# arpg/Kangaroo

Measured on AMD Instinct MI355X. Metric: kinectfusion_frames_per_sec_640x480_to_512cubed_tsdf, higher is better.
Workload: dtype f32

## Files before the change

include/kfx_debug.h:

```cpp
#ifndef KFX_DEBUG_H
#define KFX_DEBUG_H

#include "kfx.h"

#ifdef __cplusplus
extern "C" {
#endif

int kfx_debug_rmw(const kfx_volume* vol, int variant, kfx_stream stream);

int kfx_debug_div_uniform_check(float b, unsigned long long* d_out, kfx_stream stream);

int kfx_debug_div_core_check(unsigned seed, int per_divisor, unsigned long long* d_out, kfx_stream stream);
int kfx_debug_sqrt_core_check(unsigned long long* d_out, kfx_stream stream);
int kfx_debug_wave_xor_check(unsigned seed, unsigned long long* d_out, kfx_stream stream);

int kfx_debug_summary_export(kfx_sdf_summary* s, float tol, float vref, int fine_shift, void* R_out, void* C_out, int dims_out[12],
                             kfx_stream stream);


#ifdef __cplusplus
}
#endif
#endif
```

kangaroo_amd/csrc/debug.hip:

```cpp
#include "kfx_device.h"
#include "sampling.h"
#include "../../include/kfx_debug.h"

namespace kfx {

__global__ __launch_bounds__(256) void k_rmw_linear(float4* __restrict__ base, size_t n4)
{
    const size_t stride = (size_t)gridDim.x * blockDim.x;
    for (size_t i = (size_t)blockIdx.x * blockDim.x + threadIdx.x; i < n4; i += stride) {
        float4 c = base[i];
        c.y += 1.0f;
        c.w += 1.0f;
        base[i] = c;
    }
}

template <int ZC>
__global__ __launch_bounds__(256) void k_rmw_brick(unsigned char* vptr, size_t pitch, size_t img_pitch, int X, int Y, int Z)
{
    const int tid = threadIdx.x, lane = tid & 63, wv = tid >> 6;
    const int x0 = (blockIdx.x * 32 + (lane & 31)) * 2;
    const int y = blockIdx.y * 8 + wv * 2 + (lane >> 5);
    const int zbeg = blockIdx.z * ZC, zend = min(zbeg + ZC, Z);
    if (x0 >= X || y >= Y) return;
// ... 173 lines not shown
    hipLaunchKernelGGL(k_div_core_check, dim3(4096), dim3(256), 0, (hipStream_t)stream, seed, per_divisor, d_out);
    return check_launch("kfx_debug_div_core_check");
}

extern "C" int kfx_debug_sqrt_core_check(unsigned long long* d_out, kfx_stream stream)
{
    if (!d_out) return set_error(KFX_E_NULL, "kfx_debug_sqrt_core_check");
    hipLaunchKernelGGL(k_sqrt_core_check, dim3(4096), dim3(256), 0, (hipStream_t)stream, d_out);
    return check_launch("kfx_debug_sqrt_core_check");
}

extern "C" int kfx_debug_div_uniform_check(float b, unsigned long long* d_out, kfx_stream stream)
{
    if (!d_out) return set_error(KFX_E_NULL, "kfx_debug_div_uniform_check");
    if (!div_uniform_safe_host(b)) return set_error(KFX_E_RANGE, "kfx_debug_div_uniform_check: divisor outside [2^-40, 2^40]");
    hipLaunchKernelGGL(k_div_uniform_check, dim3(256), dim3(256), 0, (hipStream_t)stream, b, 1.0f / b, d_out);
    return check_launch("kfx_debug_div_uniform_check");
}

extern "C" int kfx_debug_rmw(const kfx_volume* vol, int variant, kfx_stream stream)
{
    if (!vol || !vol->ptr) return set_error(KFX_E_NULL, "kfx_debug_rmw");
    hipStream_t s = (hipStream_t)stream;
    const int X = (int)vol->w, Y = (int)vol->h, Z = (int)vol->d;
    unsigned char* p = (unsigned char*)vol->ptr;
    switch (variant) {
    case 0: {
        const size_t n4 = ((vol->d - 1) * vol->img_pitch + (vol->h - 1) * vol->pitch + vol->w * 8) / 16;
        hipLaunchKernelGGL(k_rmw_linear, dim3(256 * 8), dim3(256), 0, s, (float4*)p, n4);
        break;
    }
    case 1: hipLaunchKernelGGL(k_rmw_brick<16>, dim3(ceil_div(X, 64), ceil_div(Y, 8), ceil_div(Z, 16)), dim3(256), 0, s, p, vol->pitch, vol->img_pitch, X, Y, Z); break;
    case 2: hipLaunchKernelGGL(k_rmw_rows<16>, dim3(ceil_div(X, 128), ceil_div(Y, 4), ceil_div(Z, 16)), dim3(256), 0, s, p, vol->pitch, vol->img_pitch, X, Y, Z); break;
    case 3: hipLaunchKernelGGL(k_rmw_column, dim3(ceil_div(X, 128), ceil_div(Y, 4), 1), dim3(256), 0, s, p, vol->pitch, vol->img_pitch, X, Y, Z); break;
    case 4: hipLaunchKernelGGL(k_rmw_brick<64>, dim3(ceil_div(X, 64), ceil_div(Y, 8), ceil_div(Z, 64)), dim3(256), 0, s, p, vol->pitch, vol->img_pitch, X, Y, Z); break;
    case 5: hipLaunchKernelGGL(k_rmw_rows<4>, dim3(ceil_div(X, 128), ceil_div(Y, 4), ceil_div(Z, 4)), dim3(256), 0, s, p, vol->pitch, vol->img_pitch, X, Y, Z); break;
#define GEN(ID, WX, WY, ZC, NT) \
    case ID: hipLaunchKernelGGL((k_rmw_gen<WX, WY, ZC, NT>), dim3(ceil_div(X, 128 * WX), ceil_div(Y, WY), ceil_div(Z, ZC)), dim3(256), 0, s, p, vol->pitch, vol->img_pitch, X, Y, Z); break;
    GEN(10, 4, 1, 16, false)
    GEN(11, 2, 2, 16, false)
    GEN(12, 1, 4, 16, false)
    GEN(13, 1, 4, 16, true)
    GEN(14, 4, 1, 16, true)
    GEN(15, 1, 4, 1, false)
    GEN(16, 1, 4, 64, false)
    GEN(17, 4, 1, 4, false)
    GEN(18, 2, 2, 16, true)
#undef GEN
    default: return set_error(KFX_E_RANGE, "kfx_debug_rmw: variant");
    }
    return check_launch("kfx_debug_rmw");
}

extern "C" int kfx_debug_summary_export(kfx_sdf_summary* s, float tol, float vref, int fine_shift, void* R_out, void* C_out, int dims_out[12],
                                        kfx_stream stream)
{
    if (!s || !dims_out) return set_error(KFX_E_NULL, "kfx_debug_summary_export: null argument");
    if (fine_shift < 3 || fine_shift > 5) return set_error(KFX_E_RANGE, "kfx_debug_summary_export: fine_shift in [3, 5]");
    ClassView cv;
    summary_class_layout(s, fine_shift, cv);
    dims_out[0] = s->nbx; dims_out[1] = s->nby; dims_out[2] = s->nbz;
    dims_out[3] = cv.fine.first; dims_out[4] = cv.fine.rw; dims_out[5] = cv.fine.ny;
    dims_out[6] = cv.coarse.first; dims_out[7] = cv.coarse.rw; dims_out[8] = cv.coarse.ny;
    dims_out[9] = cv.words; dims_out[10] = s->n_coarse; dims_out[11] = (s->h_skippable && s->builds) ? ((volatile int*)s->h_skippable)[(s->builds - 1) % KFX_SUMMARY_RING] : -2;
    const size_t n = (size_t)s->nbx * s->nby * s->nbz;
    hipStream_t st = (hipStream_t)stream;
    if (R_out && hipMemcpyAsync(R_out, s->R, n * sizeof(float4), hipMemcpyDeviceToDevice, st) != hipSuccess) return set_error(KFX_E_RANGE, "kfx_debug_summary_export: copy");
    if (C_out) {
        if (int e = summary_classes_prepare(s, tol, vref, fine_shift, st)) return e;
        if (hipMemcpyAsync(C_out, s->C, (size_t)cv.words * sizeof(unsigned), hipMemcpyDeviceToDevice, st) != hipSuccess || hipStreamSynchronize(st) != hipSuccess)
            return set_error(KFX_E_RANGE, "kfx_debug_summary_export: copy");
        dims_out[11] = (s->h_skippable && s->builds) ? ((volatile int*)s->h_skippable)[(s->builds - 1) % KFX_SUMMARY_RING] : -2;
    }
    return 0;
}
```

kangaroo_amd/csrc/host_args.h:

```cpp
#pragma once

#include <cstdio>
#include <cstdlib>

#include "kfx_device.h"

namespace kfx {

constexpr size_t VOLUME_MAX_DIM = 65535, VOLUME_ANY_DIM = ~(size_t)0;

inline int check_volume(const kfx_volume* vol, size_t cell_bytes, size_t min_dim, size_t max_dim, const char* what)
{
    auto fail = [what](int code, const char* rule) {
        char msg[160];
        snprintf(msg, sizeof(msg), "%s: %s", what, rule);
        return set_error(code, msg);
    };
    if (!vol || !vol->ptr) return fail(KFX_E_NULL, "null volume");
    if (vol->w < min_dim || vol->h < min_dim || vol->d < min_dim || vol->w > max_dim || vol->h > max_dim || vol->d > max_dim)
        return fail(KFX_E_SHAPE, "volume dimensions");
    if (vol->pitch < vol->w * cell_bytes || vol->img_pitch < vol->pitch * (vol->h - 1) + vol->w * cell_bytes)
        return fail(KFX_E_SHAPE, "volume pitch smaller than a row / slice");
    if (((uintptr_t)vol->ptr | vol->pitch | vol->img_pitch) & (cell_bytes - 1)) return fail(KFX_E_ALIGN, "volume not aligned to its cell size");
    return 0;
}

inline kfx_volume slab_full_volume(const kfx_volume* vol, const kfx_slab* slab)
{
    kfx_volume full = *vol;
    full.ptr = (unsigned char*)vol->ptr - (ptrdiff_t)slab->z_offset * (ptrdiff_t)vol->img_pitch;
    full.d = slab->full_d;
    full.boxmin[2] = slab->full_zmin;
    full.boxmax[2] = slab->full_zmax;
    return full;
}

inline int env_int(const char* name, int dflt)
{
    const char* e = getenv(name);
    return e ? atoi(e) : dflt;
}
inline int env_int(const char* name, int dflt, int lo, int hi)
{
    const int v = env_int(name, dflt);
    return v < lo ? lo : (v > hi ? hi : v);
}
inline float env_float(const char* name, float dflt)
{
    const char* e = getenv(name);
    return e ? (float)atof(e) : dflt;
}

}
```

kangaroo_amd/csrc/kfx_device.h:

```cpp
#pragma once

#include <hip/hip_runtime.h>
#include <stddef.h>
#include <stdint.h>

#include "../../include/kfx.h"
#include "../../include/kfx_extras.h"
#include "../../include/kfx_summary_h.h"

namespace kfx {

struct V3 { float x, y, z; };

__device__ __forceinline__ V3 v3(float x, float y, float z) { return V3{x, y, z}; }
__device__ __forceinline__ V3 operator+(V3 a, V3 b) { return V3{a.x + b.x, a.y + b.y, a.z + b.z}; }
__device__ __forceinline__ V3 operator-(V3 a, V3 b) { return V3{a.x - b.x, a.y - b.y, a.z - b.z}; }
__device__ __forceinline__ V3 operator*(V3 a, float s) { return V3{a.x * s, a.y * s, a.z * s}; }
__device__ __forceinline__ V3 div_cw(V3 a, V3 b) { return V3{a.x / b.x, a.y / b.y, a.z / b.z}; }
__device__ __forceinline__ V3 div_s(V3 a, float s) { const float inv = 1.0f / s; return a * inv; }
__device__ __forceinline__ float dot(V3 a, V3 b) { return a.x * b.x + a.y * b.y + a.z * b.z; }
__device__ __forceinline__ float length(V3 a) { return sqrtf(dot(a, a)); }
__device__ __forceinline__ float lerp(float a, float b, float t) { return a + t * (b - a); }
__device__ __forceinline__ V3 lerp(V3 a, V3 b, float t) { return a + (b - a) * t; }
__device__ __forceinline__ float clampf(float f, float a, float b) { return fmaxf(a, fminf(f, b)); }
// ... 73 lines not shown
__device__ __forceinline__ V3 se3_mul(const Pose& T, V3 p)
{
    return V3{T.m[0] * p.x + T.m[1] * p.y + T.m[2] * p.z + T.m[3],
              T.m[4] * p.x + T.m[5] * p.y + T.m[6] * p.z + T.m[7],
              T.m[8] * p.x + T.m[9] * p.y + T.m[10] * p.z + T.m[11]};
}
__device__ __forceinline__ V3 so3_mul(const Pose& T, V3 r)
{
    return V3{T.m[0] * r.x + T.m[1] * r.y + T.m[2] * r.z,
              T.m[4] * r.x + T.m[5] * r.y + T.m[6] * r.z,
              T.m[8] * r.x + T.m[9] * r.y + T.m[10] * r.z};
}
__device__ __forceinline__ V3 so3_mul_inv(const Pose& T, V3 r)
{
    return V3{T.m[0] * r.x + T.m[4] * r.y + T.m[8] * r.z,
              T.m[1] * r.x + T.m[5] * r.y + T.m[9] * r.z,
              T.m[2] * r.x + T.m[6] * r.y + T.m[10] * r.z};
}

struct ImgView {
    const unsigned char* ptr;
    size_t pitch;
    int w, h;
};
template <typename T>
__device__ __forceinline__ const T* row(const ImgView& im, size_t y)
{
    return reinterpret_cast<const T*>(im.ptr + y * im.pitch);
}

struct VolView {
    unsigned char* ptr;
    size_t pitch, img_pitch;
    int w, h, d;
    V3 bmin, bmax;
};

__host__ __device__ inline int ceil_div(int a, int b) { return (a + b - 1) / b; }

}

#define KFX_SUMMARY_RING 8
struct kfx_sdf_summary {
    float4* R;
    int nbx, nby, nbz;
    int w, h, d;
    int cell_bytes;
    const unsigned char* base;
    size_t pitch, img_pitch;
    unsigned* C;
    int c_dirty;
    float c_tol, c_vref;
    int c_shift;
    int c_global;
    int n_coarse;
    int* d_count;
    int* h_skippable;
    int* d_skippable;
    hipEvent_t build_done[8];
    unsigned builds;
    unsigned plain_calls;
    unsigned sweeps;
};
namespace kfx {
struct ClassLevel {
    int shift;
    int ny;
    int rw;
    int first;
};
struct ClassView {
    const unsigned* C;
    ClassLevel fine, coarse;
    int words;
    float vref;
    float tol;
    int amb_ok;
    int ox, oy, oz;
    float eps;
    int nx5, nz5, top_n, lds_words;
    int global, top_first, stage_words;
};
inline __host__ __device__ void class_level_up(const int nx, const int ny, const int nz, const int shift, const int first, ClassLevel& L, int& ux, int& uz, int& words)
{
    ux = (nx + 1) >> 1; uz = (nz + 1) >> 1;
    L.shift = shift; L.ny = (ny + 1) >> 1; L.rw = 2 * ((ux + 31) >> 5); L.first = first;
    words = (L.rw * L.ny * uz + 3) & ~3;
}
int summary_classes_prepare(kfx_sdf_summary* s, float tol, float vref, int fine_shift, hipStream_t stream, int global = 0);
void summary_class_layout(const kfx_sdf_summary* s, int fine_shift, ClassView& cv);
void summary_top_layout(const ClassView& cv, ClassLevel& l6, ClassLevel& l7, int& w6, int& w7);
int summary_view_offset(const kfx_sdf_summary* s, const kfx_volume* view, int* ox, int* oy, int* oz);
}

namespace kfx {
int set_error(int code, const char* what);
int check_launch(const char* what);
int math_mode();
size_t texel_image_bytes(size_t w, size_t h);
int depth_to_vbo_normals_texels(const kfx_image* vbo, const kfx_image* nrm, const kfx_image* depth, const float K[4], float scale,
                                const kfx_image* texels, kfx_stream stream);
int sdf_fuse_slab_texels(const kfx_volume* vol, const kfx_slab* slab, const kfx_image* depth, const kfx_image* norm, const kfx_image* texels,
                         const float T_cw[12], const float K[4], float trunc_dist, float max_w, float mincostheta, unsigned flags, kfx_stream stream);
int sdf_fuse_texels(const kfx_volume* vol, kfx_sdf_summary* summary, const kfx_image* depth, const kfx_image* norm, const kfx_image* texels,
                    const float T_cw[12], const float K[4], float trunc_dist, float max_w, float mincostheta, unsigned flags, kfx_stream stream);
}
```

kangaroo_amd/csrc/raycast.hip:

```cpp
#include <cmath>

#include <hip/hip_fp16.h>

#include "kfx_device.h"
#include "sampling.h"

namespace kfx {

struct RayParams {
    VolView vol;
    V3 size;
    V3 dims1;
    V3 hi2;
    V3 voxel;
    V3 inv_size;
    int fastdiv, off32;
    Pose T;
    Intr K;
    unsigned char *dptr, *nptr, *iptr;
    size_t dpitch, npitch, ipitch;
    int w, h;
    float near, far, trunc;
    int subpix;
    int tile_log2w;
// ... 753 lines not shown
template <typename CELL>
static int class_view(ClassView& cl, size_t* lds_bytes, int* usable, kfx_sdf_summary* summary, const kfx_volume* vol, const RayParams& p, kfx_stream stream,
                      bool allow_global = true)
{
    *usable = 0;
    if (int e = summary_view_offset(summary, vol, &cl.ox, &cl.oy, &cl.oz)) return e;
    if (!(p.trunc > 0.f) || !(p.trunc < __builtin_inff())) return 0;
    static const int kb_env = env_int("KFX_RAYCAST_CLASS_KB", 16, 1, 60);
    static const int gt_env = env_int("KFX_RAYCAST_GLOBAL_TABLES", 0);
    static const int top_env = env_int("KFX_RAYCAST_TOP_LEVELS", 2, 0, 2);
    int fine = 3;
    for (; fine < 5; ++fine) {
        summary_class_layout(summary, fine, cl);
        if ((size_t)cl.words * 4 <= (size_t)kb_env * 1024) break;
    }
    auto top_levels = [&](int& w6, int& w7) {
        summary_class_layout(summary, fine, cl);
        cl.nx5 = ceil_div(summary->w, 32); cl.nz5 = ceil_div(summary->d, 32);
        ClassLevel l6, l7;
        summary_top_layout(cl, l6, l7, w6, w7);
        const int nx6 = (cl.nx5 + 1) >> 1, nz6 = (cl.nz5 + 1) >> 1;
        cl.top_n = 0;
        if (cl.nx5 > 1 || cl.coarse.ny > 1 || cl.nz5 > 1) cl.top_n = 1;
        if (cl.top_n && (nx6 > 1 || l6.ny > 1 || nz6 > 1)) cl.top_n = 2;
        if (cl.top_n > top_env) cl.top_n = top_env;
    };
    int w6, w7;
    top_levels(w6, w7);
    const size_t lds_static = sizeof(RayParams) + sizeof(TopLevels) + 2048;
    const int derived = (cl.top_n > 0 ? w6 : 0) + (cl.top_n > 1 ? w7 : 0);
    cl.global = gt_env > 0 || (size_t)cl.words * 4 > 60 * 1024 || (size_t)(cl.words + derived) * 4 + lds_static > 64 * 1024;
    if (cl.global) {
        fine = 4;
        top_levels(w6, w7);
        cl.top_first = cl.words;
        cl.stage_words = (cl.top_n > 0 ? w6 : 0) + (cl.top_n > 1 ? w7 : 0);
        cl.lds_words = cl.stage_words;
        if ((size_t)cl.lds_words * 4 + lds_static > 64 * 1024) return 0;
    } else {
        cl.top_first = 0;
        cl.stage_words = cl.words;
        cl.lds_words = cl.words + derived;
    }
    if (cl.global && !allow_global) return 0;
    const bool half = CELL::BYTES == 4;
    const float vref = half ? __half2float(__float2half_rn(p.trunc)) : p.trunc;
    const float tol = math_mode() == KFX_MATH_FAST ? (half ? KFX_SUMMARY_HALF_BAND : 1e-5f) : 0.f;
    static const int force_env = env_int("KFX_RAYCAST_SUMMARY", 0);
    if (force_env < 0) return 0;
    const bool steer = force_env == 0 && summary->h_skippable;
    if (steer && summary->plain_calls && (summary->plain_calls++ % 8u) != 0u) return 0;
    if (int e = summary_classes_prepare(summary, tol, vref, fine, (hipStream_t)stream, cl.global)) return e;
    if (steer && summary->builds >= 3) {
        const unsigned ref = (summary->builds - 3) % KFX_SUMMARY_RING;
        (void)hipEventSynchronize(summary->build_done[ref]);
        const int known = ((volatile int*)summary->h_skippable)[ref];
        if (known >= 0 && (long long)known * 4 < summary->n_coarse) {
            if (!summary->plain_calls) summary->plain_calls = 1;
            return 0;
        }
        summary->plain_calls = 0;
    }
    cl.C = summary->C;
    cl.vref = vref;
    cl.amb_ok = fmaxf(vref, p.voxel.x) == p.trunc ? 1 : 0;
    cl.tol = tol;
    const double u24 = 1.0 / 16777216.0;
    double eps = 0.0;
    const float bmin[3] = {p.vol.bmin.x, p.vol.bmin.y, p.vol.bmin.z}, bmax[3] = {p.vol.bmax.x, p.vol.bmax.y, p.vol.bmax.z};
    const float size[3] = {p.size.x, p.size.y, p.size.z}, dims1[3] = {p.dims1.x, p.dims1.y, p.dims1.z};
    const float cw[3] = {p.T.m[3], p.T.m[7], p.T.m[11]};
    for (int a = 0; a < 3; ++a) {
        if (!(size[a] > 0.f)) return 0;
        const double sc = (double)dims1[a] / size[a];
        const double pmax = std::fmax(std::fabs((double)bmin[a]), std::fabs((double)bmax[a])), ca = std::fabs((double)cw[a]);
        const double A = std::fabs(((double)cw[a] - bmin[a]) * sc);
        const double t = sc * (3.0 * pmax + 2.0 * ca + size[a]) * u24 + 2.0 * dims1[a] * u24;
        const double e = u24 * (3.0 * A + 2.0 * sc * (pmax + ca) + dims1[a]) + 3.0 * u24 * (dims1[a] + A);
        eps = std::fmax(eps, t + e);
    }
    eps *= 2.0;
    if (!(eps < 0.05)) return 0;
    cl.eps = (float)std::fmax(eps, 1e-4);
    *lds_bytes = (size_t)cl.lds_words * sizeof(unsigned);
    *usable = 1;
    return 0;
}

template <typename CELL>
static int raycast_levels_launch(int n_levels, const kfx_image* const* depth, const kfx_image* const* norm, const kfx_image* const* img,
                                 const kfx_image* const* vbo, const kfx_volume* vol, const float T_wc[12], const float* K, float near, float far,
                                 float trunc_dist, int subpix, kfx_stream stream, kfx_sdf_summary* summary = nullptr)
{
    if (n_levels < 0 || n_levels > RAY_MAX_LEVELS) return set_error(KFX_E_RANGE, "RaycastSdf(levels): number of levels");
    if (!depth || !norm || !img || !K) return set_error(KFX_E_NULL, "RaycastSdf(levels): null argument");
    RayParams base{};
    RayLevels L{};
    int blocks = 0;
    for (int l = 0; l < n_levels; ++l) {
        RayParams p;
        if (int e = ray_params<CELL>(p, depth[l], norm[l], img[l], vol, T_wc, K + 4 * l, near, far, trunc_dist, subpix)) return e;
        if (p.w == 0 || p.h == 0) continue;
        RayLevel& lv = L.lv[L.n++];
        lv.dptr = p.dptr; lv.nptr = p.nptr; lv.iptr = p.iptr;
        lv.dpitch = p.dpitch; lv.npitch = p.npitch; lv.ipitch = p.ipitch;
        lv.w = p.w; lv.h = p.h;
        lv.K = p.K;
        lv.vptr = nullptr;
        lv.vpitch = 0;
// ... 303 lines not shown
```

kangaroo_amd/csrc/summary.hip:

```cpp
#include <algorithm>
#include <new>

#include <hip/hip_fp16.h>

#include "kfx_device.h"

namespace kfx {

__global__ __launch_bounds__(256) void k_summary_fill(float4* __restrict__ R, size_t n, float lo, float hi, int state)
{
    const size_t i = (size_t)blockIdx.x * 256 + threadIdx.x;
    if (i < n) R[i] = make_float4(lo, hi, __int_as_float(state), 0.f);
}

struct ClassBuild {
    const float4* R;
    unsigned* C;
    int nbx, nby, nbz;
    int shift, nx, ny, nz, rw;
    float lo_ok, hi_ok;
    const unsigned* src;
    int src_shift, src_nx, src_ny, src_nz, src_rw;
};
template <int M>
__device__ __forceinline__ int class_row(const ClassBuild& b, const long long wave)
{
    const float4* __restrict__ R = b.R;
    unsigned* __restrict__ C = b.C;
    const unsigned* __restrict__ src = b.src;
    const int nbx = b.nbx, nby = b.nby, nbz = b.nbz, shift = b.shift, nx = b.nx, ny = b.ny, rw = b.rw;
    const int src_shift = b.src_shift, src_nx = b.src_nx, src_ny = b.src_ny, src_nz = b.src_nz, src_rw = b.src_rw;
    const float lo_ok = b.lo_ok, hi_ok = b.hi_ok;
    const int lane = threadIdx.x & 63;
    const int chunks = (nx + 63) >> 6;
    const int chunk = (int)(wave % chunks), by = (int)((wave / chunks) % ny), bz = (int)(wave / ((long long)chunks * ny));
    const int bx = chunk * 64 + lane;
    int cls = 0;
    if (bx < nx) {
        bool all_nan = true, all_free = true, all_either = true;
        if constexpr (M == 0) {
            const int m = 1 << (shift - src_shift);
            for (int z0 = 0; z0 < m; z0 += 2) {
                uint2 w2[2][4];
#pragma unroll
                for (int dz = 0; dz < 2; ++dz)
#pragma unroll
                    for (int dy = 0; dy < 4; ++dy) {
                        const int z = min(bz * m + z0 + dz, src_nz - 1), y = min(by * m + min(dy, m - 1), src_ny - 1);
                        w2[dz][dy] = *reinterpret_cast<const uint2*>(src + ((size_t)z * src_ny + y) * src_rw + (((bx * m) >> 5) << 1));
                    }
#pragma unroll
                for (int dz = 0; dz < 2; ++dz)
#pragma unroll
                    for (int dy = 0; dy < 4; ++dy)
                        for (int dx = 0; dx < m; ++dx) {
                            const int x = min(bx * m + dx, src_nx - 1);
                            const int c = (int)((w2[dz][dy].x >> (x & 31)) & 1u) | (int)(((w2[dz][dy].y >> (x & 31)) & 1u) << 1);
                            all_free = all_free && c == 1;
                            all_nan = all_nan && c == 2;
                            all_either = all_either && c != 0;
                        }
            }
        } else if constexpr (M > 2) {
            for (int z = bz * M; z <= bz * M + M; ++z)
                for (int y = by * M; y <= by * M + M; ++y)
                    for (int x = bx * M; x <= bx * M + M; ++x) {
                        const float4 r = R[((size_t)min(z, nbz - 1) * nby + min(y, nby - 1)) * nbx + min(x, nbx - 1)];
                        const int st = __float_as_int(r.z);
                        const bool in_band = r.x >= lo_ok && r.y <= hi_ok;
                        all_nan = all_nan && st == 1;
                        all_free = all_free && st == 0 && in_band;
                        all_either = all_either && (st == 1 || in_band);
                    }
        } else {
            float4 r[(M + 1) * (M + 1) * (M + 1)];
#pragma unroll
            for (int dz = 0; dz <= M; ++dz)
#pragma unroll
                for (int dy = 0; dy <= M; ++dy)
#pragma unroll
                    for (int dx = 0; dx <= M; ++dx)
                        r[(dz * (M + 1) + dy) * (M + 1) + dx] =
                            R[((size_t)min(bz * M + dz, nbz - 1) * nby + min(by * M + dy, nby - 1)) * nbx + min(bx * M + dx, nbx - 1)];
#pragma unroll
            for (int k = 0; k < (M + 1) * (M + 1) * (M + 1); ++k) {
                const int st = __float_as_int(r[k].z);
                const bool in_band = r[k].x >= lo_ok && r[k].y <= hi_ok;
                all_nan = all_nan && st == 1;
                all_free = all_free && st == 0 && in_band;
                all_either = all_either && (st == 1 || in_band);
            }
        }
        cls = all_free ? 1 : (all_nan ? 2 : (all_either ? 3 : 0));
    }
    const unsigned long long p0 = __ballot(cls & 1), p1 = __ballot(cls & 2);
    if (lane == 0) {
        unsigned* row = C + ((size_t)bz * ny + by) * rw + chunk * 4;
        row[0] = (unsigned)p0; row[1] = (unsigned)p1;
        if (chunk * 4 + 2 < rw) { row[2] = (unsigned)(p0 >> 32); row[3] = (unsigned)(p1 >> 32); }
    }
    return __popcll(p0 | p1);
}

template <int M>
__global__ __launch_bounds__(256) void k_summary_classes(const ClassBuild b, const long long n_waves)
{
    const long long wave = (long long)blockIdx.x * 4 + (threadIdx.x >> 6);
    if (wave < n_waves) class_row<M>(b, wave);
}

template <int M>
__global__ __launch_bounds__(256) void k_summary_classes_coarse(const ClassBuild b, const long long n_waves, int* __restrict__ count, int* __restrict__ publish)
{
    __shared__ int s_count[4];
    const int wv = threadIdx.x >> 6;
    const long long wave = (long long)blockIdx.x * 4 + wv;
    const int n = wave < n_waves ? class_row<M>(b, wave) : 0;
    if ((threadIdx.x & 63) == 0) s_count[wv] = n;
    __syncthreads();
    if (threadIdx.x == 0) {
        atomicAdd(&count[0], s_count[0] + s_count[1] + s_count[2] + s_count[3]);
        __threadfence();
        if (atomicAdd(&count[1], 1) == (int)gridDim.x - 1) {
            __threadfence();
            const int total = atomicExch(&count[0], 0);
            count[1] = 0;
            __hip_atomic_store(publish, total, __ATOMIC_RELAXED, __HIP_MEMORY_SCOPE_SYSTEM);
        }
    }
}

template <int BYTES>
__global__ __launch_bounds__(256) void k_summary_rebuild(float4* __restrict__ R, const unsigned char* __restrict__ base, size_t pitch, size_t img_pitch,
                                                         int w, int h, int d, int nbx, int nby, int nbz, int aligned16)
{
    const long long brick = (long long)blockIdx.x * 4 + (threadIdx.x >> 6);
    if (brick >= (long long)nbx * nby * nbz) return;
    const int lane = threadIdx.x & 63;
    const int bx = (int)(brick % nbx), by = (int)((brick / nbx) % nby), bz = (int)(brick / ((long long)nbx * nby));
    const int y = by * 8 + (lane & 7), z = bz * 8 + (lane >> 3), x0 = bx * 8;
    float lo = __builtin_inff(), hi = -__builtin_inff();
    bool nan = false, val = false;
    if (y < h && z < d) {
        const unsigned char* row = base + (size_t)z * img_pitch + (size_t)y * pitch + (size_t)x0 * BYTES;
        if (BYTES == 4 && x0 + 8 <= w && aligned16) {
            uint4 c[2];
#pragma unroll
            for (int k = 0; k < 2; ++k) c[k] = reinterpret_cast<const uint4*>(row)[k];
#pragma unroll
            for (int k = 0; k < 2; ++k) {
                const unsigned u[4] = {c[k].x, c[k].y, c[k].z, c[k].w};
#pragma unroll
                for (int j = 0; j < 4; ++j) {
                    const float a = __half2float(__ushort_as_half((unsigned short)(u[j] & 0xffffu)));
                    nan = nan || a != a;
                    val = val || a == a;
                    lo = fminf(lo, a);
                    hi = fmaxf(hi, a);
                }
            }
        } else if (BYTES == 8 && x0 + 8 <= w && aligned16) {
            float4 c[4];
#pragma unroll
            for (int k = 0; k < 4; ++k) c[k] = reinterpret_cast<const float4*>(row)[k];
#pragma unroll
            for (int k = 0; k < 4; ++k) {
                const float a = c[k].x, b = c[k].z;
                nan = nan || a != a || b != b;
                val = val || a == a || b == b;
                lo = fminf(lo, fminf(a, b));
                hi = fmaxf(hi, fmaxf(a, b));
            }
        } else {
            const int x1 = x0 + 8 < w ? x0 + 8 : w;
            for (int x = x0; x < x1; ++x) {
                const float a = BYTES == 8 ? *reinterpret_cast<const float*>(row + (size_t)(x - x0) * 8)
                                           : __half2float(__ushort_as_half(*reinterpret_cast<const unsigned short*>(row + (size_t)(x - x0) * 4)));
                nan = nan || a != a;
                val = val || a == a;
                lo = fminf(lo, a);
                hi = fmaxf(hi, a);
            }
        }
    }
    const auto fmin2 = [](float a, float b) { return fminf(a, b); };
    const auto fmax2 = [](float a, float b) { return fmaxf(a, b); };
    lo = wave_xor_combine<1>(lo, fmin2); hi = wave_xor_combine<1>(hi, fmax2);
    lo = wave_xor_combine<2>(lo, fmin2); hi = wave_xor_combine<2>(hi, fmax2);
#pragma unroll
    for (int off = 4; off <= 8; off <<= 1) { lo = fminf(lo, __shfl_xor(lo, off, 64)); hi = fmaxf(hi, __shfl_xor(hi, off, 64)); }
    lo = wave_xor_combine<16>(lo, fmin2); hi = wave_xor_combine<16>(hi, fmax2);
    lo = wave_xor_combine<32>(lo, fmin2); hi = wave_xor_combine<32>(hi, fmax2);
    const bool any_nan = __ballot(nan) != 0ull, any_val = __ballot(val) != 0ull;
    if (lane == 0) R[brick] = make_float4(lo, hi, __int_as_float(any_val ? (any_nan ? 2 : 0) : 1), 0.f);
}

static void class_level(ClassLevel& L, int shift, int w, int h, int first)
{
    L.shift = shift;
    L.ny = ceil_div(h, 1 << shift);
    L.rw = 2 * ceil_div(ceil_div(w, 1 << shift), 32);
    L.first = first;
}
static int class_level_words(const ClassLevel& L, int d) { return L.rw * L.ny * ceil_div(d, 1 << L.shift); }

void summary_class_layout(const kfx_sdf_summary* s, int fine_shift, ClassView& cv)
{
    class_level(cv.fine, fine_shift, s->w, s->h, 0);
    const int fw = fine_shift < 5 ? class_level_words(cv.fine, s->d) : 0;
    class_level(cv.coarse, 5, s->w, s->h, (fw + 3) & ~3);
    cv.words = cv.coarse.first + ((class_level_words(cv.coarse, s->d) + 3) & ~3);
}

void summary_top_layout(const ClassView& cv, ClassLevel& l6, ClassLevel& l7, int& w6, int& w7)
{
    int nx6, nz6, nx7, nz7;
    class_level_up(cv.nx5, cv.coarse.ny, cv.nz5, 6, cv.words, l6, nx6, nz6, w6);
    class_level_up(nx6, l6.ny, nz6, 7, cv.words + w6, l7, nx7, nz7, w7);
}

int summary_classes_prepare(kfx_sdf_summary* s, float tol, float vref, int fine_shift, hipStream_t stream, int global)
{
    if (!s->c_dirty && s->c_tol == tol && s->c_vref == vref && s->c_shift == fine_shift && s->c_global == global) return 0;
    ClassView cv;
    summary_class_layout(s, fine_shift, cv);
    cv.nx5 = ceil_div(s->w, 32); cv.nz5 = ceil_div(s->d, 32);
    ClassLevel l6, l7;
    int w6, w7;
    summary_top_layout(cv, l6, l7, w6, w7);
    const float lo_ok = vref - tol * vref, hi_ok = vref + tol * vref;
    for (int pass = 0; pass < (global ? 4 : 2); ++pass) {
        if (pass >= 2) {
            const ClassLevel& L = pass == 2 ? l6 : l7;
            const ClassLevel& S = pass == 2 ? cv.coarse : l6;
            ClassBuild b;
            b.R = s->R; b.C = s->C + L.first;
            b.nbx = s->nbx; b.nby = s->nby; b.nbz = s->nbz;
            b.shift = L.shift; b.nx = ceil_div(s->w, 1 << L.shift); b.ny = L.ny; b.nz = ceil_div(s->d, 1 << L.shift); b.rw = L.rw;
            b.lo_ok = lo_ok; b.hi_ok = hi_ok;
            b.src = s->C + S.first;
            b.src_shift = S.shift; b.src_nx = ceil_div(s->w, 1 << S.shift); b.src_ny = S.ny; b.src_nz = ceil_div(s->d, 1 << S.shift); b.src_rw = S.rw;
            const long long waves = (long long)ceil_div(b.nx, 64) * b.ny * b.nz;
            hipLaunchKernelGGL(k_summary_classes<0>, dim3((unsigned)((waves + 3) / 4)), dim3(256), 0, stream, b, waves);
            if (int e = check_launch("kfx_sdf_summary (classes)")) return e;
            continue;
        }
        const ClassLevel& L = pass ? cv.coarse : cv.fine;
        if (!pass && fine_shift >= 5) continue;
        ClassBuild b;
        b.R = s->R; b.C = s->C + L.first;
        b.nbx = s->nbx; b.nby = s->nby; b.nbz = s->nbz;
        b.shift = L.shift; b.nx = ceil_div(s->w, 1 << L.shift); b.ny = L.ny; b.nz = ceil_div(s->d, 1 << L.shift); b.rw = L.rw;
        b.lo_ok = lo_ok; b.hi_ok = hi_ok;
        const bool from_fine = pass && fine_shift < 5;
        b.src = from_fine ? s->C + cv.fine.first : nullptr;
        b.src_shift = cv.fine.shift; b.src_nx = ceil_div(s->w, 1 << cv.fine.shift); b.src_ny = cv.fine.ny;
        b.src_nz = ceil_div(s->d, 1 << cv.fine.shift); b.src_rw = cv.fine.rw;
        const long long waves = (long long)ceil_div(b.nx, 64) * b.ny * b.nz;
        if (pass) {
            const dim3 grid((unsigned)((waves + 3) / 4));
            const unsigned slot = s->builds % KFX_SUMMARY_RING;
            int* publish = s->d_skippable + (s->h_skippable ? slot : 0);
            if (from_fine) hipLaunchKernelGGL(k_summary_classes_coarse<0>, grid, dim3(256), 0, stream, b, waves, s->d_count, publish);
            else hipLaunchKernelGGL(k_summary_classes_coarse<4>, grid, dim3(256), 0, stream, b, waves, s->d_count, publish);
            if (s->h_skippable) (void)hipEventRecord(s->build_done[slot], stream);
            s->builds += 1;
        } else if (L.shift == 3) {
            hipLaunchKernelGGL(k_summary_classes<1>, dim3((unsigned)((waves + 3) / 4)), dim3(256), 0, stream, b, waves);
        } else {
            hipLaunchKernelGGL(k_summary_classes<2>, dim3((unsigned)((waves + 3) / 4)), dim3(256), 0, stream, b, waves);
        }
        if (int e = check_launch("kfx_sdf_summary (classes)")) return e;
    }
    s->c_dirty = 0; s->c_tol = tol; s->c_vref = vref; s->c_shift = fine_shift; s->c_global = global;
    return 0;
}

int summary_view_offset(const kfx_sdf_summary* s, const kfx_volume* view, int* ox, int* oy, int* oz)
{
    if (!s || !view || !view->ptr) return set_error(KFX_E_NULL, "summary: null argument");
    if (view->pitch != s->pitch || view->img_pitch != s->img_pitch) return set_error(KFX_E_SHAPE, "summary: the volume is not a view of the summary's volume (pitches)");
    const unsigned char* q = static_cast<const unsigned char*>(view->ptr);
    if (q < s->base) return set_error(KFX_E_SHAPE, "summary: the volume is not a view of the summary's volume");
    const size_t off = (size_t)(q - s->base);
    const size_t z = off / s->img_pitch, rem = off % s->img_pitch, y = rem / s->pitch, xb = rem % s->pitch;
    const size_t cb = (size_t)s->cell_bytes;
    if (xb % cb || z + view->d > (size_t)s->d || y + view->h > (size_t)s->h || xb / cb + view->w > (size_t)s->w)
        return set_error(KFX_E_SHAPE, "summary: the volume is not a view of the summary's volume (extent)");
    *ox = (int)(xb / cb); *oy = (int)y; *oz = (int)z;
    return 0;
}

}

using namespace kfx;

static int summary_create(kfx_sdf_summary** out, const kfx_volume* vol, int cell_bytes)
{
    if (!out || !vol || !vol->ptr) return set_error(KFX_E_NULL, "kfx_sdf_summary_create: null argument");
    if (vol->w < 2 || vol->h < 2 || vol->d < 2 || vol->w > 65535 || vol->h > 65535 || vol->d > 65535) return set_error(KFX_E_SHAPE, "kfx_sdf_summary_create: volume dimensions");
    kfx_sdf_summary* s = new (std::nothrow) kfx_sdf_summary;
    if (!s) return set_error(KFX_E_RANGE, "kfx_sdf_summary_create: out of memory");
    s->nbx = ceil_div((int)vol->w, 8); s->nby = ceil_div((int)vol->h, 8); s->nbz = ceil_div((int)vol->d, 8);
    s->w = (int)vol->w; s->h = (int)vol->h; s->d = (int)vol->d;
    s->cell_bytes = cell_bytes;
    s->base = static_cast<const unsigned char*>(vol->ptr);
    s->pitch = vol->pitch; s->img_pitch = vol->img_pitch;
    s->R = nullptr; s->C = nullptr; s->d_count = nullptr; s->h_skippable = nullptr; s->d_skippable = nullptr;
    s->c_dirty = 1; s->c_tol = -1.f; s->c_vref = 0.f; s->c_shift = 0; s->c_global = 0; s->sweeps = 0;
    s->builds = 0; s->plain_calls = 0;
    for (auto& e : s->build_done) e = nullptr;
    s->n_coarse = ceil_div(s->w, 32) * ceil_div(s->h, 32) * ceil_div(s->d, 32);
    const size_t n = (size_t)s->nbx * s->nby * s->nbz;
    ClassView cv;
    summary_class_layout(s, 3, cv);
    ClassView cg;
    summary_class_layout(s, 4, cg);
    cg.nx5 = ceil_div(s->w, 32); cg.nz5 = ceil_div(s->d, 32);
    ClassLevel l6, l7;
    int w6, w7;
    summary_top_layout(cg, l6, l7, w6, w7);
    const int words = std::max(cv.words, cg.words + w6 + w7);
    bool ok = hipMalloc((void**)&s->R, n * sizeof(float4)) == hipSuccess && hipMalloc((void**)&s->C, (size_t)words * sizeof(unsigned)) == hipSuccess &&
              hipMalloc((void**)&s->d_count, 2 * sizeof(int)) == hipSuccess && hipMemset(s->d_count, 0, 2 * sizeof(int)) == hipSuccess;
    if (ok && hipHostMalloc((void**)&s->h_skippable, KFX_SUMMARY_RING * sizeof(int), hipHostMallocMapped) == hipSuccess) {
        for (int i = 0; i < KFX_SUMMARY_RING; ++i) s->h_skippable[i] = -1;
        bool evs = hipHostGetDevicePointer((void**)&s->d_skippable, s->h_skippable, 0) == hipSuccess;
        for (int i = 0; evs && i < KFX_SUMMARY_RING; ++i) evs = hipEventCreateWithFlags(&s->build_done[i], hipEventDisableTiming) == hipSuccess;
        if (!evs) {
            for (auto& e : s->build_done) { if (e) (void)hipEventDestroy(e); e = nullptr; }
            (void)hipHostFree(s->h_skippable);
            s->h_skippable = nullptr;
        }
    } else {
        s->h_skippable = nullptr;
    }
    if (ok && !s->h_skippable) {
        (void)hipGetLastError();
        ok = hipMalloc((void**)&s->d_skippable, sizeof(int)) == hipSuccess;
    }
    if (!ok) {
        (void)hipGetLastError();
        kfx_sdf_summary_destroy(s);
        return set_error(KFX_E_NODEVICE, "kfx_sdf_summary_create: hipMalloc");
    }
    *out = s;
    return kfx_sdf_summary_invalidate(s, nullptr);
}

extern "C" int kfx_sdf_summary_create(kfx_sdf_summary** out, const kfx_volume* vol) { return summary_create(out, vol, 8); }
extern "C" int kfx_sdf_summary_create_h(kfx_sdf_summary** out, const kfx_volume* vol) { return summary_create(out, vol, 4); }

extern "C" int kfx_sdf_summary_destroy(kfx_sdf_summary* s)
{
    if (!s) return 0;
    (void)hipDeviceSynchronize();
    if (s->R) (void)hipFree(s->R);
    if (s->C) (void)hipFree(s->C);
    if (s->d_count) (void)hipFree(s->d_count);
    for (auto& e : s->build_done) if (e) (void)hipEventDestroy(e);
    if (s->h_skippable) (void)hipHostFree(s->h_skippable);
    else if (s->d_skippable) (void)hipFree(s->d_skippable);
    delete s;
    return 0;
}

extern "C" int kfx_sdf_summary_rebuild(kfx_sdf_summary* s, kfx_stream stream)
{
    if (!s) return set_error(KFX_E_NULL, "kfx_sdf_summary_rebuild: null summary");
    const long long n = (long long)s->nbx * s->nby * s->nbz;
    const int aligned16 = ((((uintptr_t)s->base) | s->pitch | s->img_pitch) & 15) == 0;
    if (s->cell_bytes == 4)
        hipLaunchKernelGGL(k_summary_rebuild<4>, dim3((unsigned)((n + 3) / 4)), dim3(256), 0, (hipStream_t)stream, s->R, s->base, s->pitch, s->img_pitch,
                           s->w, s->h, s->d, s->nbx, s->nby, s->nbz, aligned16);
    else
        hipLaunchKernelGGL(k_summary_rebuild<8>, dim3((unsigned)((n + 3) / 4)), dim3(256), 0, (hipStream_t)stream, s->R, s->base, s->pitch, s->img_pitch,
                           s->w, s->h, s->d, s->nbx, s->nby, s->nbz, aligned16);
    s->c_dirty = 1;
    return check_launch("kfx_sdf_summary_rebuild");
}

extern "C" int kfx_sdf_summary_invalidate(kfx_sdf_summary* s, kfx_stream stream)
{
    if (!s) return set_error(KFX_E_NULL, "kfx_sdf_summary_invalidate: null summary");
    const size_t n = (size_t)s->nbx * s->nby * s->nbz;
    hipLaunchKernelGGL(k_summary_fill, dim3((unsigned)((n + 255) / 256)), dim3(256), 0, (hipStream_t)stream, s->R, n, -__builtin_inff(), __builtin_inff(), 2);
    s->c_dirty = 1;
    return check_launch("kfx_sdf_summary_invalidate");
}

static int reset_tracked(const kfx_volume* vol, kfx_sdf_summary* s, float trunc_dist, kfx_stream stream, int cell_bytes, const char* name)
{
    if (!s) return set_error(KFX_E_NULL, cell_bytes == 4 ? "kfx_sdf_reset_tracked_h: null summary" : "kfx_sdf_reset_tracked: null summary");
    if (s->cell_bytes != cell_bytes) return set_error(KFX_E_SHAPE, "SdfReset(tracked): the summary was created for the other cell type");
    int ox, oy, oz;
    if (int e = summary_view_offset(s, vol, &ox, &oy, &oz)) return e;
    if (ox || oy || oz || (int)vol->w != s->w || (int)vol->h != s->h || (int)vol->d != s->d)
        return set_error(KFX_E_SHAPE, "kfx_sdf_reset_tracked: resets the whole volume only (use kfx_sdf_reset + kfx_sdf_summary_invalidate for views)");
    if (int e = cell_bytes == 4 ? kfx_sdf_reset_h(vol, trunc_dist, stream) : kfx_sdf_reset(vol, trunc_dist, stream)) return e;
    const size_t n = (size_t)s->nbx * s->nby * s->nbz;
    const bool nan = trunc_dist != trunc_dist;
    const float v = cell_bytes == 4 ? __half2float(__float2half_rn(trunc_dist)) : trunc_dist;
    hipLaunchKernelGGL(k_summary_fill, dim3((unsigned)((n + 255) / 256)), dim3(256), 0, (hipStream_t)stream, s->R, n,
                       nan ? __builtin_inff() : v, nan ? -__builtin_inff() : v, nan ? 1 : 0);
    s->c_dirty = 1;
    return check_launch(name);
}

extern "C" int kfx_sdf_reset_tracked(const kfx_volume* vol, kfx_sdf_summary* s, float trunc_dist, kfx_stream stream)
{
    return reset_tracked(vol, s, trunc_dist, stream, 8, "kfx_sdf_reset_tracked");
}

// ... 5 lines not shown
```

Measured before the change: 2406.

## Fuse fine and coarse summary class builds and replace event sync with stamped host polling

Adds a single fused kernel that classifies fine 16-cube rows and reduces them directly into coarse 32-cube classes in shared memory, replacing two separate launches when fine_shift is 4. The per-build completion count is now published as a 64-bit stamped word in mapped host memory, using a single packed atomic in place of two atomics plus fences. The host reads it by spin-polling the stamp instead of calling hipEventSynchronize, so event creation and recording are removed. This is meant to cut launch count and host synchronisation overhead in the raycast steering path. In exchange the host may busy-spin, and it falls back to stream and then device synchronisation when the stamp is missing.

```diff
diff --git a/include/kfx_debug.h b/include/kfx_debug.h
--- a/include/kfx_debug.h
+++ b/include/kfx_debug.h
@@ -18,6 +18,7 @@
 int kfx_debug_summary_export(kfx_sdf_summary* s, float tol, float vref, int fine_shift, void* R_out, void* C_out, int dims_out[12],
                              kfx_stream stream);
 
+int kfx_debug_summary_steering(const kfx_sdf_summary* s, int state_out[4]);
 
 #ifdef __cplusplus
 }
diff --git a/kangaroo_amd/csrc/debug.hip b/kangaroo_amd/csrc/debug.hip
--- a/kangaroo_amd/csrc/debug.hip
+++ b/kangaroo_amd/csrc/debug.hip
@@ -249,6 +249,13 @@
     return check_launch("kfx_debug_rmw");
 }
 
+static int last_published(const kfx_sdf_summary* s)
+{
+    if (!s->h_skippable || !s->builds) return -2;
+    const unsigned long long v = __atomic_load_n(s->h_skippable + (s->builds - 1) % KFX_SUMMARY_RING, __ATOMIC_ACQUIRE);
+    return (unsigned)(v >> 32) == s->builds ? (int)(unsigned)v : -1;
+}
+
 extern "C" int kfx_debug_summary_export(kfx_sdf_summary* s, float tol, float vref, int fine_shift, void* R_out, void* C_out, int dims_out[12],
                                         kfx_stream stream)
 {
@@ -259,7 +266,7 @@
     dims_out[0] = s->nbx; dims_out[1] = s->nby; dims_out[2] = s->nbz;
     dims_out[3] = cv.fine.first; dims_out[4] = cv.fine.rw; dims_out[5] = cv.fine.ny;
     dims_out[6] = cv.coarse.first; dims_out[7] = cv.coarse.rw; dims_out[8] = cv.coarse.ny;
-    dims_out[9] = cv.words; dims_out[10] = s->n_coarse; dims_out[11] = (s->h_skippable && s->builds) ? ((volatile int*)s->h_skippable)[(s->builds - 1) % KFX_SUMMARY_RING] : -2;
+    dims_out[9] = cv.words; dims_out[10] = s->n_coarse; dims_out[11] = last_published(s);
     const size_t n = (size_t)s->nbx * s->nby * s->nbz;
     hipStream_t st = (hipStream_t)stream;
     if (R_out && hipMemcpyAsync(R_out, s->R, n * sizeof(float4), hipMemcpyDeviceToDevice, st) != hipSuccess) return set_error(KFX_E_RANGE, "kfx_debug_summary_export: copy");
@@ -267,7 +274,15 @@
         if (int e = summary_classes_prepare(s, tol, vref, fine_shift, st)) return e;
         if (hipMemcpyAsync(C_out, s->C, (size_t)cv.words * sizeof(unsigned), hipMemcpyDeviceToDevice, st) != hipSuccess || hipStreamSynchronize(st) != hipSuccess)
             return set_error(KFX_E_RANGE, "kfx_debug_summary_export: copy");
-        dims_out[11] = (s->h_skippable && s->builds) ? ((volatile int*)s->h_skippable)[(s->builds - 1) % KFX_SUMMARY_RING] : -2;
+        dims_out[11] = last_published(s);
     }
     return 0;
 }
+
+extern "C" int kfx_debug_summary_steering(const kfx_sdf_summary* s, int state_out[4])
+{
+    if (!s || !state_out) return set_error(KFX_E_NULL, "kfx_debug_summary_steering: null argument");
+    state_out[0] = (int)s->builds; state_out[1] = (int)s->plain_calls; state_out[2] = last_published(s);
+    state_out[3] = s->c_launches;
+    return 0;
+}
diff --git a/kangaroo_amd/csrc/host_args.h b/kangaroo_amd/csrc/host_args.h
--- a/kangaroo_amd/csrc/host_args.h
+++ b/kangaroo_amd/csrc/host_args.h
@@ -51,4 +51,13 @@
     return e ? (float)atof(e) : dflt;
 }
 
+inline void cpu_pause()
+{
+#if defined(__x86_64__) || defined(__i386__)
+    __builtin_ia32_pause();
+#elif defined(__aarch64__)
+    __asm__ __volatile__("yield");
+#endif
 }
+
+}
diff --git a/kangaroo_amd/csrc/kfx_device.h b/kangaroo_amd/csrc/kfx_device.h
--- a/kangaroo_amd/csrc/kfx_device.h
+++ b/kangaroo_amd/csrc/kfx_device.h
@@ -149,17 +149,19 @@
     int c_dirty;
     float c_tol, c_vref;
     int c_shift;
+    int c_launches;
     int c_global;
     int n_coarse;
-    int* d_count;
-    int* h_skippable;
-    int* d_skippable;
-    hipEvent_t build_done[8];
+    unsigned long long* d_count;
+    unsigned long long* h_skippable;
+    unsigned long long* d_skippable;
     unsigned builds;
     unsigned plain_calls;
     unsigned sweeps;
 };
 namespace kfx {
+__host__ __device__ inline unsigned long long summary_slot(unsigned stamp, int count) { return ((unsigned long long)stamp << 32) | (unsigned)count; }
+int summary_published_count(const kfx_sdf_summary* s, unsigned build, hipStream_t stream);
 struct ClassLevel {
     int shift;
     int ny;
diff --git a/kangaroo_amd/csrc/raycast.hip b/kangaroo_amd/csrc/raycast.hip
--- a/kangaroo_amd/csrc/raycast.hip
+++ b/kangaroo_amd/csrc/raycast.hip
@@ -829,9 +829,7 @@
     if (steer && summary->plain_calls && (summary->plain_calls++ % 8u) != 0u) return 0;
     if (int e = summary_classes_prepare(summary, tol, vref, fine, (hipStream_t)stream, cl.global)) return e;
     if (steer && summary->builds >= 3) {
-        const unsigned ref = (summary->builds - 3) % KFX_SUMMARY_RING;
-        (void)hipEventSynchronize(summary->build_done[ref]);
-        const int known = ((volatile int*)summary->h_skippable)[ref];
+        const int known = summary_published_count(summary, summary->builds - 3, (hipStream_t)stream);
         if (known >= 0 && (long long)known * 4 < summary->n_coarse) {
             if (!summary->plain_calls) summary->plain_calls = 1;
             return 0;
diff --git a/kangaroo_amd/csrc/summary.hip b/kangaroo_amd/csrc/summary.hip
--- a/kangaroo_amd/csrc/summary.hip
+++ b/kangaroo_amd/csrc/summary.hip
@@ -3,6 +3,7 @@
 
 #include <hip/hip_fp16.h>
 
+#include "host_args.h"
 #include "kfx_device.h"
 
 namespace kfx {
@@ -23,7 +24,7 @@
     int src_shift, src_nx, src_ny, src_nz, src_rw;
 };
 template <int M>
-__device__ __forceinline__ int class_row(const ClassBuild& b, const long long wave)
+__device__ __forceinline__ int class_row(const ClassBuild& b, const long long wave, unsigned long long& p0, unsigned long long& p1)
 {
     const float4* __restrict__ R = b.R;
     unsigned* __restrict__ C = b.C;
@@ -93,7 +94,7 @@
         }
         cls = all_free ? 1 : (all_nan ? 2 : (all_either ? 3 : 0));
     }
-    const unsigned long long p0 = __ballot(cls & 1), p1 = __ballot(cls & 2);
+    p0 = __ballot(cls & 1); p1 = __ballot(cls & 2);
     if (lane == 0) {
         unsigned* row = C + ((size_t)bz * ny + by) * rw + chunk * 4;
         row[0] = (unsigned)p0; row[1] = (unsigned)p1;
@@ -101,6 +102,12 @@
     }
     return __popcll(p0 | p1);
 }
+template <int M>
+__device__ __forceinline__ int class_row(const ClassBuild& b, const long long wave)
+{
+    unsigned long long p0, p1;
+    return class_row<M>(b, wave, p0, p1);
+}
 
 template <int M>
 __global__ __launch_bounds__(256) void k_summary_classes(const ClassBuild b, const long long n_waves)
@@ -109,8 +116,18 @@
     if (wave < n_waves) class_row<M>(b, wave);
 }
 
+__device__ __forceinline__ void publish_count(unsigned long long* __restrict__ count, const int n, unsigned long long* __restrict__ publish, const unsigned stamp)
+{
+    const unsigned long long before = atomicAdd(count, (1ull << 32) | (unsigned)n);
+    if ((unsigned)(before >> 32) == gridDim.x - 1) {
+        *count = 0ull;
+        __hip_atomic_store(publish, summary_slot(stamp, (int)(unsigned)before + n), __ATOMIC_RELAXED, __HIP_MEMORY_SCOPE_SYSTEM);
+    }
+}
+
 template <int M>
-__global__ __launch_bounds__(256) void k_summary_classes_coarse(const ClassBuild b, const long long n_waves, int* __restrict__ count, int* __restrict__ publish)
+__global__ __launch_bounds__(256) void k_summary_classes_coarse(const ClassBuild b, const long long n_waves, unsigned long long* __restrict__ count,
+                                                                unsigned long long* __restrict__ publish, const unsigned stamp)
 {
     __shared__ int s_count[4];
     const int wv = threadIdx.x >> 6;
@@ -118,16 +135,69 @@
     const int n = wave < n_waves ? class_row<M>(b, wave) : 0;
     if ((threadIdx.x & 63) == 0) s_count[wv] = n;
     __syncthreads();
-    if (threadIdx.x == 0) {
-        atomicAdd(&count[0], s_count[0] + s_count[1] + s_count[2] + s_count[3]);
-        __threadfence();
-        if (atomicAdd(&count[1], 1) == (int)gridDim.x - 1) {
-            __threadfence();
-            const int total = atomicExch(&count[0], 0);
-            count[1] = 0;
-            __hip_atomic_store(publish, total, __ATOMIC_RELAXED, __HIP_MEMORY_SCOPE_SYSTEM);
-        }
-    }
+    if (threadIdx.x == 0) publish_count(count, s_count[0] + s_count[1] + s_count[2] + s_count[3], publish, stamp);
+}
+
+#ifndef KFX_PAIR_ROWS
+#define KFX_PAIR_ROWS 2
+#endif
+constexpr int PAIR_ROWS = KFX_PAIR_ROWS;
+__global__ __launch_bounds__(256 * PAIR_ROWS) void k_summary_classes_pair(const ClassBuild b, unsigned* __restrict__ C5, const int nx5, const int ny5, const int rw5,
+                                                                          unsigned long long* __restrict__ count, unsigned long long* __restrict__ publish,
+                                                                          const unsigned stamp)
+{
+    __shared__ unsigned long long s_plane[4 * PAIR_ROWS][2];
+    __shared__ int s_n[PAIR_ROWS];
+    const int lane = threadIdx.x & 63, wv = threadIdx.x >> 6, sub = wv >> 2;
+    const int chunks = (b.nx + 63) >> 6, groups = (ny5 + PAIR_ROWS - 1) / PAIR_ROWS;
+    const int chunk = (int)(blockIdx.x % chunks), j = (int)((blockIdx.x / chunks) % groups) * PAIR_ROWS + sub, k = (int)(blockIdx.x / ((unsigned)chunks * groups));
+    const int by = 2 * j + (wv & 1), bz = 2 * k + ((wv >> 1) & 1);
+    if (by < b.ny && bz < b.nz) {
+        unsigned long long p0, p1;
+        class_row<2>(b, ((long long)bz * b.ny + by) * chunks + chunk, p0, p1);
+        if (lane == 0) { s_plane[wv][0] = p0; s_plane[wv][1] = p1; }
+    }
+    __syncthreads();
+    int n = 0;
+    if ((wv & 3) == 0 && j < ny5) {
+        const int cx = chunk * 32 + lane;
+        int cls = 0;
+        if (lane < 32 && cx < nx5) {
+            bool all_nan = true, all_free = true, all_either = true;
+#pragma unroll
+            for (int dz = 0; dz < 2; ++dz)
+#pragma unroll
+                for (int dy = 0; dy < 2; ++dy) {
+                    const int row = 4 * sub + (min(2 * k + dz, b.nz - 1) - 2 * k) * 2 + (min(2 * j + dy, b.ny - 1) - 2 * j);
+                    const unsigned long long q0 = s_plane[row][0], q1 = s_plane[row][1];
+#pragma unroll
+                    for (int dx = 0; dx < 2; ++dx) {
+                        const int x = min(2 * cx + dx, b.nx - 1) - chunk * 64;
+                        const int c = (int)((q0 >> x) & 1ull) | (int)(((q1 >> x) & 1ull) << 1);
+                        all_free = all_free && c == 1;
+                        all_nan = all_nan && c == 2;
+                        all_either = all_either && c != 0;
+                    }
+                }
+            cls = all_free ? 1 : (all_nan ? 2 : (all_either ? 3 : 0));
+        }
+        const unsigned long long p0 = __ballot(cls & 1), p1 = __ballot(cls & 2);
+        n = __popcll(p0 | p1);
+        if (lane == 0) {
+            unsigned* row = C5 + ((size_t)k * ny5 + j) * rw5 + chunk * 2;
+            row[0] = (unsigned)p0; row[1] = (unsigned)p1;
+        }
+    }
+    if constexpr (PAIR_ROWS > 1) {
+        if ((wv & 3) == 0 && lane == 0) s_n[sub] = n;
+        __syncthreads();
+        if (threadIdx.x == 0) {
+            n = 0;
+#pragma unroll
+            for (int r = 0; r < PAIR_ROWS; ++r) n += s_n[r];
+        }
+    }
+    if (threadIdx.x == 0) publish_count(count, n, publish, stamp);
 }
 
 template <int BYTES>
@@ -229,6 +299,25 @@
     int w6, w7;
     summary_top_layout(cv, l6, l7, w6, w7);
     const float lo_ok = vref - tol * vref, hi_ok = vref + tol * vref;
+    const unsigned slot = s->builds % KFX_SUMMARY_RING, stamp = s->builds + 1;
+    unsigned long long* publish = s->d_skippable + (s->h_skippable ? slot : 0);
+    static const int pair_env = env_int("KFX_SUMMARY_PAIR_BUILD", 1);
+    if (pair_env && fine_shift == 4 && !global) {
+        ClassBuild b{};
+        b.R = s->R; b.C = s->C + cv.fine.first;
+        b.nbx = s->nbx; b.nby = s->nby; b.nbz = s->nbz;
+        b.shift = 4; b.nx = ceil_div(s->w, 16); b.ny = cv.fine.ny; b.nz = ceil_div(s->d, 16); b.rw = cv.fine.rw;
+        b.lo_ok = lo_ok; b.hi_ok = hi_ok;
+        const long long groups = (long long)ceil_div(b.nx, 64) * ceil_div(cv.coarse.ny, PAIR_ROWS) * cv.nz5;
+        hipLaunchKernelGGL(k_summary_classes_pair, dim3((unsigned)groups), dim3(256 * PAIR_ROWS), 0, stream, b, s->C + cv.coarse.first, cv.nx5, cv.coarse.ny, cv.coarse.rw,
+                           s->d_count, publish, stamp);
+        s->builds += 1;
+        s->c_launches = 1;
+        if (int e = check_launch("kfx_sdf_summary (classes)")) return e;
+        s->c_dirty = 0; s->c_tol = tol; s->c_vref = vref; s->c_shift = fine_shift; s->c_global = global;
+        return 0;
+    }
+    s->c_launches = 0;
     for (int pass = 0; pass < (global ? 4 : 2); ++pass) {
         if (pass >= 2) {
             const ClassLevel& L = pass == 2 ? l6 : l7;
@@ -243,6 +332,7 @@
             const long long waves = (long long)ceil_div(b.nx, 64) * b.ny * b.nz;
             hipLaunchKernelGGL(k_summary_classes<0>, dim3((unsigned)((waves + 3) / 4)), dim3(256), 0, stream, b, waves);
             if (int e = check_launch("kfx_sdf_summary (classes)")) return e;
+            s->c_launches += 1;
             continue;
         }
         const ClassLevel& L = pass ? cv.coarse : cv.fine;
@@ -259,11 +349,8 @@
         const long long waves = (long long)ceil_div(b.nx, 64) * b.ny * b.nz;
         if (pass) {
             const dim3 grid((unsigned)((waves + 3) / 4));
-            const unsigned slot = s->builds % KFX_SUMMARY_RING;
-            int* publish = s->d_skippable + (s->h_skippable ? slot : 0);
-            if (from_fine) hipLaunchKernelGGL(k_summary_classes_coarse<0>, grid, dim3(256), 0, stream, b, waves, s->d_count, publish);
-            else hipLaunchKernelGGL(k_summary_classes_coarse<4>, grid, dim3(256), 0, stream, b, waves, s->d_count, publish);
-            if (s->h_skippable) (void)hipEventRecord(s->build_done[slot], stream);
+            if (from_fine) hipLaunchKernelGGL(k_summary_classes_coarse<0>, grid, dim3(256), 0, stream, b, waves, s->d_count, publish, stamp);
+            else hipLaunchKernelGGL(k_summary_classes_coarse<4>, grid, dim3(256), 0, stream, b, waves, s->d_count, publish, stamp);
             s->builds += 1;
         } else if (L.shift == 3) {
             hipLaunchKernelGGL(k_summary_classes<1>, dim3((unsigned)((waves + 3) / 4)), dim3(256), 0, stream, b, waves);
@@ -271,9 +358,27 @@
             hipLaunchKernelGGL(k_summary_classes<2>, dim3((unsigned)((waves + 3) / 4)), dim3(256), 0, stream, b, waves);
         }
         if (int e = check_launch("kfx_sdf_summary (classes)")) return e;
+        s->c_launches += 1;
     }
     s->c_dirty = 0; s->c_tol = tol; s->c_vref = vref; s->c_shift = fine_shift; s->c_global = global;
     return 0;
+}
+
+int summary_published_count(const kfx_sdf_summary* s, unsigned build, hipStream_t stream)
+{
+    if (!s->h_skippable) return -1;
+    unsigned long long* word = s->h_skippable + build % KFX_SUMMARY_RING;
+    const unsigned stamp = build + 1;
+    for (int attempt = 0; attempt < 3; ++attempt) {
+        for (int spin = 0; spin < (attempt ? 1 : 1 << 14); ++spin) {
+            const unsigned long long v = __atomic_load_n(word, __ATOMIC_ACQUIRE);
+            if ((unsigned)(v >> 32) == stamp) return (int)(unsigned)v;
+            cpu_pause();
+        }
+        if (attempt == 0) (void)hipStreamSynchronize(stream);
+        else if (attempt == 1) (void)hipDeviceSynchronize();
+    }
+    return -1;
 }
 
 int summary_view_offset(const kfx_sdf_summary* s, const kfx_volume* view, int* ox, int* oy, int* oz)
@@ -307,9 +412,8 @@
     s->base = static_cast<const unsigned char*>(vol->ptr);
     s->pitch = vol->pitch; s->img_pitch = vol->img_pitch;
     s->R = nullptr; s->C = nullptr; s->d_count = nullptr; s->h_skippable = nullptr; s->d_skippable = nullptr;
-    s->c_dirty = 1; s->c_tol = -1.f; s->c_vref = 0.f; s->c_shift = 0; s->c_global = 0; s->sweeps = 0;
+    s->c_dirty = 1; s->c_tol = -1.f; s->c_vref = 0.f; s->c_shift = 0; s->c_global = 0; s->c_launches = 0; s->sweeps = 0;
     s->builds = 0; s->plain_calls = 0;
-    for (auto& e : s->build_done) e = nullptr;
     s->n_coarse = ceil_div(s->w, 32) * ceil_div(s->h, 32) * ceil_div(s->d, 32);
     const size_t n = (size_t)s->nbx * s->nby * s->nbz;
     ClassView cv;
@@ -322,13 +426,10 @@
     summary_top_layout(cg, l6, l7, w6, w7);
     const int words = std::max(cv.words, cg.words + w6 + w7);
     bool ok = hipMalloc((void**)&s->R, n * sizeof(float4)) == hipSuccess && hipMalloc((void**)&s->C, (size_t)words * sizeof(unsigned)) == hipSuccess &&
-              hipMalloc((void**)&s->d_count, 2 * sizeof(int)) == hipSuccess && hipMemset(s->d_count, 0, 2 * sizeof(int)) == hipSuccess;
-    if (ok && hipHostMalloc((void**)&s->h_skippable, KFX_SUMMARY_RING * sizeof(int), hipHostMallocMapped) == hipSuccess) {
-        for (int i = 0; i < KFX_SUMMARY_RING; ++i) s->h_skippable[i] = -1;
-        bool evs = hipHostGetDevicePointer((void**)&s->d_skippable, s->h_skippable, 0) == hipSuccess;
-        for (int i = 0; evs && i < KFX_SUMMARY_RING; ++i) evs = hipEventCreateWithFlags(&s->build_done[i], hipEventDisableTiming) == hipSuccess;
-        if (!evs) {
-            for (auto& e : s->build_done) { if (e) (void)hipEventDestroy(e); e = nullptr; }
+              hipMalloc((void**)&s->d_count, sizeof(unsigned long long)) == hipSuccess && hipMemset(s->d_count, 0, sizeof(unsigned long long)) == hipSuccess;
+    if (ok && hipHostMalloc((void**)&s->h_skippable, KFX_SUMMARY_RING * sizeof(unsigned long long), hipHostMallocMapped) == hipSuccess) {
+        for (int i = 0; i < KFX_SUMMARY_RING; ++i) s->h_skippable[i] = 0ull;
+        if (hipHostGetDevicePointer((void**)&s->d_skippable, s->h_skippable, 0) != hipSuccess) {
             (void)hipHostFree(s->h_skippable);
             s->h_skippable = nullptr;
         }
@@ -337,7 +438,7 @@
     }
     if (ok && !s->h_skippable) {
         (void)hipGetLastError();
-        ok = hipMalloc((void**)&s->d_skippable, sizeof(int)) == hipSuccess;
+        ok = hipMalloc((void**)&s->d_skippable, sizeof(unsigned long long)) == hipSuccess;
     }
     if (!ok) {
         (void)hipGetLastError();
@@ -358,7 +459,6 @@
     if (s->R) (void)hipFree(s->R);
     if (s->C) (void)hipFree(s->C);
     if (s->d_count) (void)hipFree(s->d_count);
-    for (auto& e : s->build_done) if (e) (void)hipEventDestroy(e);
     if (s->h_skippable) (void)hipHostFree(s->h_skippable);
     else if (s->d_skippable) (void)hipFree(s->d_skippable);
     delete s;
```

Result: no change. 2414 (median of 2 runs) (+0.3%).
